# JJanai/back2future

Measured on AMD Instinct MI355X. Metric: frame-triplets/sec at 3x1024x1920, higher is better.
Workload: dtype f32; 1 GPU; BASELINE.json configs[4] per-GPU share: batch=16 synthetic 3x1024x1920 triplets per GPU, random-init pwc.lua weights (Ours-Hard shape), outputs flow + occ + est[3]; batch_per_gpu=16, global_batch=16, height=1024, width=1920, parallelism=dp1: independent triplets per rank, one RCCL weight broadcast at init, hip_graph=True

## Files before the change

### back2future_amd/_lib.py

```python
import ctypes as C
import os

import numpy as np

_HERE = os.path.dirname(os.path.abspath(__file__))
SO_PATH = os.environ.get("B2F_LIB") or os.path.join(_HERE, "libb2f.so")
_lib = None

c_float_p = C.POINTER(C.c_float)


class LossGradOpts(C.Structure):
    _fields_ = [("smooth_flow", C.c_double), ("const_vel", C.c_double), ("pme", C.c_double), ("smooth_occ", C.c_double),
                ("prior_occ", C.c_double), ("level_weights", C.c_double * 7), ("size_average", C.c_int)]


c_grad_opts_p = C.POINTER(LossGradOpts)


class LossGradFtOpts(C.Structure):
    _fields_ = LossGradOpts._fields_ + [("smooth_second_order", C.c_int), ("pme_criterion", C.c_int), ("pme_alpha", C.c_double),
                                        ("pme_beta", C.c_double), ("pme_gamma", C.c_double)]


# ... 336 lines not shown
    "b2f_op_cv_variant": (C.c_int, [C.c_void_p, C.c_int, C.c_int, C.c_int, C.c_int, C.c_int]),
    "b2f_op_conv_first": (C.c_int, [C.c_void_p, c_float_p, C.c_int, C.c_int, C.c_int, C.c_int, c_float_p, c_float_p, c_float_p]),
    "b2f_op_conv_head16": (C.c_int, [C.c_void_p, c_float_p, C.c_int, C.c_int, C.c_int, c_float_p, c_float_p, c_float_p, c_float_p, c_float_p]),
    "b2f_op_upsample_flow2x": (C.c_int, [C.c_void_p, c_float_p, C.c_int, C.c_int, C.c_int, c_float_p]),
    "b2f_op_image_scale": (C.c_int, [C.c_void_p, c_float_p, C.c_int, C.c_int, C.c_int, C.c_int, c_float_p, C.c_int, C.c_int]),
    "b2f_op_upsample_flow2x_ex": (C.c_int, [C.c_void_p, c_float_p, C.c_int, C.c_int, C.c_int, C.c_int, C.c_int, c_float_p]),
    "b2f_op_softmax_nearest4": (C.c_int, [C.c_void_p, c_float_p, C.c_int, C.c_int, C.c_int, C.c_int, c_float_p]),
    "b2f_op_avgpool2": (C.c_int, [C.c_void_p, c_float_p, C.c_int, C.c_int, C.c_int, C.c_int, c_float_p]),
    "b2f_op_pack_input": (C.c_int, [C.c_void_p, c_float_p, C.c_int, C.c_int, C.c_int, C.c_int, c_float_p]),
    "b2f_op_warp_image": (C.c_int, [C.c_void_p, C.c_int, C.c_void_p, C.c_int, C.c_int, c_float_p, C.c_float, C.c_int, C.c_int, C.c_int, c_float_p]),
    "b2f_op_conv_first_seq": (C.c_int, [C.c_void_p, C.c_void_p, C.c_int, C.c_int, C.c_int, C.c_int, c_float_p, c_float_p, c_float_p]),
    "b2f_op_layout": (C.c_int, [C.c_void_p, C.c_int, c_float_p, C.c_int, C.c_int, C.c_int, C.c_int, C.c_int, c_float_p]),
    "b2f_op_graph_put_channels": (C.c_int, [C.c_void_p, c_float_p, C.c_int, C.c_int, C.c_int, C.c_int, C.c_int, c_float_p, C.c_int, C.c_int]),
    "b2f_op_graph_costvol": (C.c_int, [C.c_void_p, c_float_p, c_float_p, c_float_p, C.c_int, C.c_int, C.c_int, C.c_int, C.c_int, C.c_int,
                                       c_float_p, C.c_int, c_float_p, C.c_int]),
    "b2f_op_graph_warp": (C.c_int, [C.c_void_p, c_float_p, C.c_int, c_float_p, C.c_float, C.c_int, C.c_int, C.c_int, c_float_p]),
    "b2f_op_graph_add_flow": (C.c_int, [C.c_void_p, c_float_p, c_float_p, C.c_longlong]),
    "b2f_op_graph_scale": (C.c_int, [C.c_void_p, c_float_p, C.c_longlong, C.c_float]),
    "b2f_op_graph_softmax_nearest": (C.c_int, [C.c_void_p, c_float_p, C.c_int, C.c_int, C.c_int, C.c_int, c_float_p]),
    "b2f_op_expf": (C.c_int, [C.c_void_p, c_float_p, C.c_longlong, c_float_p]),
    "b2f_arena_check": (C.c_int, [C.c_void_p, C.POINTER(C.c_int), C.POINTER(C.c_longlong)]),
    "b2f_guard_selftest": (C.c_int, [C.c_void_p, C.c_int]),
    "b2f_arena_plan": (C.c_int, [C.c_int, C.c_int, C.c_int, C.c_int, C.c_int, C.POINTER(C.c_longlong), C.c_int, C.POINTER(C.c_longlong)]),
}


class B2FError(RuntimeError):
    pass


def lib():
    global _lib
    if _lib is None:
        if not os.path.exists(SO_PATH):
            raise B2FError("%s is missing: build it with `python -m back2future_amd.build` "
                           "(there is no CPU fallback for the computeFlow path)" % SO_PATH)
        L = C.CDLL(SO_PATH)
        for name, (res, args) in SIGNATURES.items():
            fn = getattr(L, name)
            fn.restype = res
            fn.argtypes = args
        _lib = L
    return _lib


def check(rc):
# ... 11 lines not shown
```

### back2future_amd/back2future.py

```python
import ctypes as C
import weakref

import numpy as np

from . import _lib

meanstd = {"mean": [0.485, 0.456, 0.406], "std": [0.229, 0.224, 0.225]}
occ_threshold = 0.6666

IN_NORMALIZED, IN_UNIT, IN_U8 = 0, 1, 2
RGB_PLANAR, RGB_PACKED = 0, 1
STREAM_WARP, STREAM_PAST = 1, 2
SCORE_PIXELS, SCORE_EPE_Q20, SCORE_OUTLIERS, SCORE_OCC, SCORE_NONFINITE, SCORE_WORDS = 0, 4, 8, 12, 21, 22
PHOTO_INSIDE, PHOTO_OUTSIDE, PHOTO_CHARB_Q30, PHOTO_SQ_Q30, PHOTO_OCHARB_Q30, PHOTO_WEIGHT_Q30, PHOTO_NONFINITE, PHOTO_WORDS = 0, 2, 4, 6, 8, 10, 12, 14
LOSS_PIXELS, LOSS_SMOOTH_FLOW_Q30, LOSS_SMOOTH_PAST_Q30, LOSS_CONST_VEL_Q30, LOSS_SMOOTH_OCC_Q30, LOSS_PRIOR_OCC_Q30 = 0, 1, 2, 3, 4, 5
LOSS_PHOTO_INSIDE, LOSS_PHOTO_OUTSIDE, LOSS_PHOTO_OCHARB_Q30, LOSS_PHOTO_NONFINITE, LOSS_NONFINITE, LOSS_WORDS = 6, 8, 10, 12, 14, 16
LOSS_LEVEL_WEIGHTS = (0.005, 0.01, 0.02, 0.08, 0.32, 0.64, 1.28)
LOSS_WEIGHTS = {"smooth_flow": 1.0, "const_vel": 1.0, "pme": 1.0, "smooth_occ": 0.1, "prior_occ": 0.1}
LOSS_FT_SMOOTH2_FLOW_Q30, LOSS_FT_SMOOTH2_PAST_Q30, LOSS_FT_PHOTO_OGX_Q30, LOSS_FT_PHOTO_OGY_Q30 = 16, 17, 18, 20
LOSS_FT_SMOOTH2_NONFINITE, LOSS_FT_GRAD_NONFINITE, LOSS_FT_WORDS = 22, 23, 24
LOSS_SSIM_Q30, LOSS_SSIM_L1N_Q30, LOSS_SSIM_NONFINITE, LOSS_SSIM_RANGE_USED, LOSS_SSIM_RANGE_OWN, LOSS_SSIM_WORDS = 16, 18, 20, 22, 24, 32
SSIM_RANGE_BATCH, SSIM_RANGE_IMAGE, SSIM_RANGE_GIVEN = 0, 1, 2
SSIM_ALPHA = {"OSSIM": 1.0, "OSSIML1": 0.85}
LOSS_PLAIN_L1_Q30, LOSS_PLAIN_SQ_Q30, LOSS_PLAIN_SSIM_Q30, LOSS_PLAIN_L1N_Q30, LOSS_PLAIN_SSIM_NONFINITE = 16, 18, 20, 22, 24
# ... 1443 lines not shown

        entry = _grad_entry("b2f_multi_forward_loss_grad", options)
        fn = lambda h, xp, n, H, W, fsc, op, lp, gp, ng, outs, *tail: entry(h, xp, n, H, W, fsc, op, lp, gp, ng, *tail)
        L = no.value // (5 if pf.value else 4)
        grad, loss, _ = _forward_loss_grad(fn, self._h, x, flow_scale, options, shapes, L, want_loss, False,
                                           _grad_range_args(options, ssim_range, L, "MultiModel.forwardLossGrad", batch_ok=False))
        return (grad, loss) if want_loss else grad


ARENA_BUFFERS = (["img", "tmp"] + ["cs[%d]" % l for l in range(2, 8)] + ["U[%d]" % l for l in range(3, 7)] + ["UB[%d]" % l for l in range(3, 7)]
                 + ["cv"] + ["d[%d]" % i for i in range(1, 6)] + ["fs", "bfs", "logits", "u2", "flow_planar"] + ["ds[%d]" % k for k in range(2, 6)])


def arena_plan(B, H, W, full=False, past_flow=False, seq=False, stream=False, want_past=False, arena_guard=0):
    off, total = (C.c_longlong * 40)(), C.c_longlong()
    flags = (1 if full else 0) | (2 if past_flow else 0) | (4 if seq else 0) | (8 if stream else 0) | (16 if want_past else 0)
    n = _lib.lib().b2f_arena_plan(int(arena_guard), int(B), int(H), int(W), flags, off, 40, C.byref(total))
    if n < 0:
        _lib.check(1)
    assert n == len(ARENA_BUFFERS)
    return dict(zip(ARENA_BUFFERS, list(off)[:n])), total.value


def shard_range(n, rank, world):
    lo, hi = C.c_int(), C.c_int()
    _lib.check(_lib.lib().b2f_shard_range(int(n), int(rank), int(world), C.byref(lo), C.byref(hi)))
    return lo.value, hi.value


def init(opt=None, device=0):
    opt = opt or "Ours-Soft-ft-KITTI"
    model = Model(opt, device)

    def computeFlow(im1, im2, im3):
        return model.computeFlow(im1, im2, im3)

    computeFlow.model = model
    return computeFlow
```

### back2future_amd/csrc/b2f_api.hip

```cpp
#include "b2f_ctx.h"

#include <cctype>
#include <cmath>
#include <cstdio>
#include <cstdlib>

using namespace b2f;

static thread_local std::string g_err;
namespace b2f {
int api_fail(const std::string &m)
{
    g_err = m;
    return 1;
}
const std::string &api_error() { return g_err; }

ConvSeg cp8_seg(const float *ptr, int C, size_t hw)
{
    ConvSeg sgm;
    sgm.ptr = ptr;
    sgm.img_stride = (long)(hw * (size_t)((C + 7) / 8 * 8));
    sgm.chunk_stride = (long)(hw * 8);
    sgm.pix_stride = 8;
// ... 415 lines not shown
        if (o.wino1d && p.has(K_W1B) && blocks > 0 && w1b_supported(L)) {
            ch.kernel = K_W1B;
            ch.w1b_blocks = blocks;
        } else if (o.wino6 && p.has(K_WINO6) && H * W >= o.wino6_min_pixels && wino6_supported(L)) {
            ch.kernel = K_WINO6;
        }
    }
    return ch;
}

}

int b2f::launch_layer(b2f_ctx *c, hipStream_t s, bool prof, const PackedConv &p, const float *wpk, const KernelOpts &o, int cur_batch, ConvLaunch &L)
{
    for (int i = 0; i < p.nseg; ++i) L.seg[i].nchunks = p.chunks[i];
    if (p.nseg == 1) L.seg[1] = L.seg[0], L.seg[1].nchunks = 0;
    L.nseg = p.nseg;
    L.cout = p.cout;
    L.Ho = (L.H + 2 - 3) / L.stride + 1;
    L.Wo = (L.W + 2 - 3) / L.stride + 1;
    L.tiles_per_block = o.s2_tiles_per_block;
    L.w4_persist = o.wino4_persistent;
    L.w8 = o.wino8;
    L.bf16_direct = o.bf16_direct;
    auto weights = [&](ConvKernel k) { return p.has(k) ? wpk + p.pk[k].w_off : nullptr; };
    auto bias = [&](ConvKernel k) { return p.has(k) ? wpk + p.pk[k].b_off : nullptr; };
    L.wpk_bf6 = weights(K_BF6); L.bias_bf6 = bias(K_BF6);
    L.wpk_s2b = weights(K_S2B); L.bias_s2b = bias(K_S2B);
    L.wpk_w1b = weights(K_W1B); L.bias_w1b = bias(K_W1B);
    L.wpk_w6 = weights(K_WINO6); L.bias_w6 = bias(K_WINO6);
    const KernelChoice ch = choose_kernel(p, o, cur_batch, L);
    const PackedConv::Packing &q = p.pk[ch.f2x2 ? K_WINO2 : p.base];
    L.wpk = wpk + q.w_off;
    L.bias = wpk + q.b_off;
    L.nt = q.nt;
    L.nblk = q.nblk;
    L.nsplit = ch.nsplit;
    L.w1b_nblk = ch.w1b_blocks;
#if B2F_EXPERIMENTS
    if (!ch.f2x2) { L.wpk_split = weights(K_WINO4S); L.wpk_split2 = weights(K_WINO2S); }
    L.w4_hybrid = o.wino4_hybrid;
#endif
    const KernelRow &k = kKernels[ch.kernel];
    char name[48];
    if (c->profile_layers)
        snprintf(name, sizeof name, "conv%s_%dto%d_%dx%d", (B2F_EXPERIMENTS && ch.kernel == K_C16 && o.bf16_direct) ? "B16" : k.tag[L.stride - 1],
// ... 304 lines not shown
    OPT_SYNC = 2,
    OPT_EXP_ONLY = 4,
    OPT_ARENA = 8,
};
struct OptRow {
    const char *name;
    int b2f_ctx::*member;
    int flags;
    int repack;
};
const OptRow kOptions[] = {
    {"use_graph", &b2f_ctx::use_graph, OPT_ENV, 0},
    {"host_graph", &b2f_ctx::host_graph, OPT_ENV, 0},
    {"profile", &b2f_ctx::profile, OPT_ENV, 0},
    {"profile_layers", &b2f_ctx::profile_layers, OPT_ENV, 0},
    {"corr_variant", &b2f_ctx::corr_variant, OPT_ENV | OPT_SYNC, 0},
    {"corr_ablate", &b2f_ctx::corr_ablate, OPT_ENV | OPT_SYNC, 0},
    {"bf16_direct", &b2f_ctx::bf16_direct, OPT_ENV | OPT_SYNC, 0},
    {"bf16_conv", &b2f_ctx::bf16_conv, OPT_ENV | OPT_SYNC, 1},
    {"bf16_conv_min_pixels", &b2f_ctx::bf16_conv_min_pixels, OPT_SYNC, 0},
    {"wino1d", &b2f_ctx::wino1d, OPT_ENV | OPT_SYNC, 2},
    {"wino6", &b2f_ctx::wino6, OPT_ENV | OPT_SYNC, 3},
    {"wino6_min_pixels", &b2f_ctx::wino6_min_pixels, OPT_ENV | OPT_SYNC, 0},
    {"wino2_split", &b2f_ctx::wino2_split, OPT_ENV | OPT_SYNC | OPT_EXP_ONLY, 4},
    {"wino4_split", &b2f_ctx::wino4_split, OPT_ENV | OPT_SYNC | OPT_EXP_ONLY, 5},
    {"wino4_hybrid", &b2f_ctx::wino4_hybrid, OPT_ENV | OPT_SYNC | OPT_EXP_ONLY, 5},
    {"s2_tiles_per_block", &b2f_ctx::s2_tiles_per_block, OPT_ENV | OPT_SYNC, 0},
    {"wino4_persistent", &b2f_ctx::wino4_persistent, OPT_ENV | OPT_SYNC, 0},
    {"s2_loader", &b2f_ctx::s2_loader, OPT_ENV | OPT_SYNC, 0},
    {"s2_tile_groups", &b2f_ctx::s2_tile_groups, OPT_ENV | OPT_SYNC, 0},
    {"wino_split_pixels", &b2f_ctx::wino_split_pixels, OPT_ENV | OPT_SYNC, 0},
    {"wino8", &b2f_ctx::wino8, OPT_ENV | OPT_SYNC, 0},
    {"wino4_min_pixels", &b2f_ctx::wino4_min_pixels, OPT_ENV | OPT_SYNC, 0},
    {"adaptive_kernels", &b2f_ctx::adaptive_kernels, OPT_ENV | OPT_SYNC, 0},
    {"op_wino_split", &b2f_ctx::op_wino_split, OPT_ENV, 0},
    {"op_gradw_partials", &b2f_ctx::op_gradw_partials, OPT_ENV, 0},
    {"op_hole_fill", &b2f_ctx::op_hole_fill, 0, 0},
    {"host_subbatch_pixels", nullptr, OPT_ENV, 0},
    {"host_threads", &b2f_ctx::host_threads, OPT_ENV, 0},
    {"host_u8", &b2f_ctx::host_u8, OPT_ENV, 0},
    {"host_ramp", &b2f_ctx::host_ramp, OPT_ENV, 0},
    {"debug_fail_next", &b2f_ctx::debug_fail_next, 0, 0},
    {"arena_guard", &b2f_ctx::arena_guard, OPT_ARENA, 0},
    {"arena_fill", &b2f_ctx::arena_fill, OPT_ARENA, 0},
};

// ... 6 lines not shown

bool reads_packing(const b2f_ctx *c, int group)
{
    for (const OptRow &r : kOptions)
        if (r.repack == group && (r.member == &b2f_ctx::bf16_conv ? c->*r.member >= 2 : c->*r.member != 0)) return true;
    return false;
}

const char *experiment_value(const OptRow &r, int value)
{
    if (B2F_EXPERIMENTS) return nullptr;
    if (r.member == &b2f_ctx::corr_variant && (value == 2 || value == 4 || value == 6 || value == 8))
        return "b2f_set_option: corr_variant 2 / 4 / 6 / 8 are experiment kernels: build with `python -m back2future_amd.build --experiments`";
    if (r.member == &b2f_ctx::bf16_direct && value == 1)
        return "b2f_set_option: bf16_direct = 1 (the 16 -> 16 layer alone on the bf16 pipe) is an experiment: build with `python -m back2future_amd.build --experiments`";
    return nullptr;
}

}

extern "C" {

const char *b2f_last_error(void) { return g_err.c_str(); }
int b2f_version(void) { return 1015; }

long long b2f_param_count(int past_flow) { return param_count(past_flow != 0); }

int b2f_random_weights(unsigned long long seed, int past_flow, float gain, float *out, long long n) try
{
    if (!out || n != param_count(past_flow != 0)) return fail("b2f_random_weights: bad buffer size");
    random_weights(seed, past_flow != 0, gain, out);
    return 0;
}
B2F_CATCH("b2f_random_weights")

int b2f_load_t7(const char *path, float *out, long long cap, long long *n, int *past_flow) try
{
    std::vector<float> flat;
    bool past = false;
    std::string err;
    if (!path) return fail("b2f_load_t7: null path");
    if (!load_t7(path, flat, past, err)) return fail("b2f_load_t7: " + err);
    if (n) *n = (long long)flat.size();
    if (past_flow) *past_flow = past ? 1 : 0;
    if (out) {
        if (cap < (long long)flat.size()) return fail("b2f_load_t7: output buffer too small");
        memcpy(out, flat.data(), flat.size() * sizeof(float));
// ... 230 lines not shown
        if (r->member == &b2f_ctx::arena_guard && (value < 0 || value % 64)) return fail("b2f_set_option: arena_guard is a count of floats, a multiple of 64");
        if (r->member == &b2f_ctx::arena_fill && value != 0 && value != 1) return fail("b2f_set_option: arena_fill is 0 or 1");
        HIPCHK(hipSetDevice(c->device));
        HIPCHK(hipDeviceSynchronize());
        drop_graphs(c);
        if (c->arena) HIPCHK(hipFree(c->arena));
        c->arena = nullptr;
        c->arena_floats = 0;
        c->guards.clear();
        c->arena_layout[0] = 0;
    }
    const bool had = r->repack && reads_packing(c, r->repack);
    c->*r->member = value;
    if (r->repack && had != reads_packing(c, r->repack)) CHK(b2f_commit_weights(c));
    return 0;
}
B2F_CATCH("b2f_set_option")

int b2f_get_option(const b2f_ctx *c, const char *key, int *value) try
{
    if (!c || !key || !value) return fail("b2f_get_option: null argument");
    const OptRow *r = find_option(key);
    if (!strcmp(key, "experiments")) *value = B2F_EXPERIMENTS;
    else if (!r) return fail(std::string("b2f_get_option: unknown key ") + key);
    else if (!r->member) *value = (int)std::min<long long>(c->host_subbatch_pixels, 0x7fffffff);
    else *value = c->*r->member;
    return 0;
}
B2F_CATCH("b2f_get_option")

int b2f_synchronize(b2f_ctx *c) try
{
    if (!c) return fail("b2f_synchronize: null context");
    HIPCHK(hipSetDevice(c->device));
    HIPCHK(hipStreamSynchronize(c->stream));
    return 0;
}
B2F_CATCH("b2f_synchronize")

int b2f_profile_reset(b2f_ctx *c) try
{
    if (!c) return fail("b2f_profile_reset: null context");
    CHK(prof_collect(c));
    std::fill(c->prof_ms.begin(), c->prof_ms.end(), 0.0);
    std::fill(c->prof_n.begin(), c->prof_n.end(), 0);
    return 0;
// ... 677 lines not shown
B2F_CATCH("b2f_guard_selftest")

int b2f_arena_plan(int arena_guard, int B, int H, int W, int flags, long long *offsets, int cap, long long *total) try
{
    if (!offsets || cap < 33 || arena_guard < 0 || arena_guard % 64) { fail("b2f_arena_plan: bad argument"); return -1; }
    if (check_shape(B, H, W)) return -1;
    const Plan p = make_plan((size_t)arena_guard, B, H, W, (flags & 1) != 0, (flags & 2) != 0, (flags & 4) != 0, (flags & 8) != 0, (flags & 16) != 0);
    int n = 0;
    offsets[n++] = (long long)p.img;
    offsets[n++] = (long long)p.tmp;
    for (int l = 2; l <= 7; ++l) offsets[n++] = (long long)p.cs[l];
    for (int l = 3; l <= 6; ++l) offsets[n++] = (long long)p.U[l];
    for (int l = 3; l <= 6; ++l) offsets[n++] = (long long)p.UB[l];
    offsets[n++] = (long long)p.cv;
    for (int i = 1; i <= 5; ++i) offsets[n++] = (long long)p.d[i];
    for (size_t o : {p.fs, p.bfs, p.logits, p.u2, p.flow_planar}) offsets[n++] = (long long)o;
    for (int k = 2; k <= 5; ++k) offsets[n++] = (long long)p.ds[k];
    if (total) *total = (long long)p.total;
    return n;
}
catch (const std::exception &e) { fail(std::string("b2f_arena_plan: ") + e.what()); return -1; }
catch (...) { fail("b2f_arena_plan: unknown exception"); return -1; }

}

int b2f::pointer_kind(const void *p)
{
    hipPointerAttribute_t a;
    if (hipPointerGetAttributes(&a, p) != hipSuccess) {
        (void)hipGetLastError();
        return 0;
    }
    if (a.type == hipMemoryTypeDevice || a.type == hipMemoryTypeManaged || a.type == hipMemoryTypeArray) return -1;
    return a.type == hipMemoryTypeHost ? 1 : 0;
}

int b2f::check_device_pointers(const std::string &w, const b2f_ctx *c, const char *use, const void *const *ptrs, size_t count, size_t aligned)
{
    uintptr_t bits = 0;
    for (size_t i = 0; i < aligned; ++i) bits |= (uintptr_t)ptrs[i];
    if (bits & 15) return fail(w + ": device buffers must be 16-byte aligned");
    if (!c) return fail(w + ": null context");
    HIPCHK(hipSetDevice(c->device));
    for (size_t i = 0; i < count; ++i)
        if (ptrs[i] && host_memory(ptrs[i])) return fail(w + ": host memory passed to a device entry point (use " + use + ")");
    return 0;
// ... 18 lines not shown
```

### back2future_amd/csrc/b2f_ctx.h

```cpp
#pragma once
#include "../../include/b2f.h"

#include <algorithm>
#include <atomic>
#include <condition_variable>
#include <cstring>
#include <deque>
#include <exception>
#include <map>
#include <memory>
#include <mutex>
#include <string>
#include <thread>
#include <tuple>
#include <vector>

#include "b2f_host.h"
#include "b2f_internal.h"

namespace b2f {

int api_fail(const std::string &m);
const std::string &api_error();

// ... 22 lines not shown
    int cout = 0;
    ConvKernel base = K_DIRECT;
    struct Packing {
        size_t w_off = 0, b_off = 0;
        int nt = 0, nblk = 0;
    } pk[K_COUNT];
    bool has(ConvKernel k) const { return pk[k].nblk != 0; }
    int nchunks() const { return chunks[0] + (nseg > 1 ? chunks[1] : 0); }
};

struct KernelOpts {
    int wino8 = 1;
    int wino_split_pixels = 512;
    int wino4_min_pixels = 4096;
    int adaptive_kernels = -1;
    int bf16_direct = 2;
    int bf16_conv_min_pixels = 65536;
    int bf16_conv = 1;
    int wino2_split = 0;
    int wino4_hybrid = 0;
    int wino4_split = 0;
    int wino6 = 1;
    int wino6_min_pixels = 16384;
    int wino1d = 0;
    int s2_tile_groups = 1;
    int s2_loader = 1;
    int wino4_persistent = 1;
    int s2_tiles_per_block = 0;
};

struct ProfEvent {
    int name;
    hipEvent_t a, b;
};

struct GraphKey {
    const void *in;
    float *flow, *occ, *est3;
    int kind, B, H, W;
    int rule;
    int seq;
    const void *ring = nullptr;
    int phase = 0;
    float *past = nullptr;
    bool operator<(const GraphKey &o) const
    {
// ... 566 lines not shown
```

### back2future_amd/csrc/b2f_internal.h

```cpp
#pragma once
#include <hip/hip_runtime.h>
#ifndef B2F_EXPERIMENTS
#define B2F_EXPERIMENTS 0
#endif
#include <atomic>
#include <cstdint>

namespace b2f {

constexpr int kLevels = 7, kLst = 3, kWin = 9, kND = 2 * kWin * kWin;
constexpr int kFeat[8] = {0, 3, 16, 32, 64, 96, 128, 192};
constexpr int kDec[7] = {0, 128, 128, 96, 64, 32, 2};
constexpr int kCvRec = 168;
constexpr int kCvChunks = 21;
constexpr int kImgC = 8;
constexpr int kCK = 8;

struct ConvSeg {
    const float *ptr;
    long img_stride;
    long chunk_stride;
    int pix_stride;
    int nchunks;
};
// ... 12 lines not shown
    int nimg;
    int leaky;
    long long *trace;
    int nb0;
    int nsplit;
    int w8 = 1;
    int w4_persist = 1;
    int tiles_per_block = 0;
    int w4_hybrid = 0;
    const void *wpk_split2 = nullptr;
    const void *wpk_bf6 = nullptr;
    const float *bias_bf6 = nullptr;
    int bf16_direct = 0;
    const void *wpk_split = nullptr;
    const void *wpk_w1b = nullptr;
    const float *bias_w1b = nullptr;
    const void *wpk_s2b = nullptr;
    const float *bias_s2b = nullptr;
    int w1b_nblk = 0;
    const void *wpk_w6 = nullptr;
    const float *bias_w6 = nullptr;
    unsigned w6_mul[3] = {0, 0, 0};
    int w6_sh[3] = {0, 0, 0};
};
hipError_t launch_conv3x3(const ConvLaunch &p, hipStream_t s);
size_t conv_wpk_floats(int cin_chunks, int nt, int nblk);
void conv_choose_tiles(int cout, int *nt, int *nblk);
void conv_pack_weights(const float *w, const float *b, int Co, int Ci, const int *cin_map,
                       int cin_chunks, int nt, int nblk, float *wpk, float *bpk);

hipError_t launch_conv3x3_c16(const ConvLaunch &p, hipStream_t s);
hipError_t launch_conv3x3_c16b(const ConvLaunch &p, hipStream_t s);
size_t c16_wpk_floats();
void c16_pack_weights(const float *w, const float *b, int Ci, const int *cin_map, float *wpk, float *bpk);
bool convb_supported(const ConvLaunch &p);
hipError_t launch_conv3x3_bf6(const ConvLaunch &p, hipStream_t s);
int convb_nblk(int cout);
size_t convb_wpk_floats(int cin_chunks, int cout);
void convb_pack_weights(const float *w, const float *b, int Co, int Ci, const int *cin_map, int cin_chunks, float *wpk, float *bpk);
bool s2b_supported(const ConvLaunch &p);
hipError_t launch_conv3x3_s2b(const ConvLaunch &p, hipStream_t s);
int s2b_ntiles(int cout);
size_t s2b_wpk_floats(int cin_chunks, int cout);
void s2b_pack_weights(const float *w, const float *b, int Co, int Ci, const int *cin_map, int cin_chunks, float *wpk, float *bpk);
bool w1b_supported(const ConvLaunch &p);
hipError_t launch_conv3x3_w1b(const ConvLaunch &p, hipStream_t s);
int w1b_nblk(int cout);
size_t w1b_wpk_floats(int cin_chunks, int cout);
void w1b_pack_weights(const float *w, const float *b, int Co, int Ci, const int *cin_map, int cin_chunks, float *wpk, float *bpk);
bool wino6_supported(const ConvLaunch &p);
hipError_t launch_conv3x3_wino6(const ConvLaunch &p, hipStream_t s);
int wino6_nblk(int cout);
size_t wino6_wpk_floats(int cin_chunks, int cout);
void wino6_pack_weights(const float *w, const float *b, int Co, int Ci, const int *cin_map, int cin_chunks, float *wpk, float *bpk);
struct HeadLaunch {
    const float *in;
    long in_img_stride, in_chunk_stride;
    int in_pix_stride;
    int H1, W1;
    const float *w1, *b1, *w2, *b2;
    float *out;
    long out_img_stride, out_chunk_stride;
    int out_pix_stride;
    int Ho, Wo, nimg;
    int rows_per_block, nsy, nsx;
    long long *trace = nullptr;
};
bool head16_supported(const HeadLaunch &p);
hipError_t launch_conv_head16(HeadLaunch p, hipStream_t s);
bool c16s2_supported(const ConvLaunch &p);
hipError_t launch_conv3x3_c16s2(const ConvLaunch &p, hipStream_t s);
size_t c16s2_wpk_floats();
void c16s2_pack_weights(const float *w, const float *b, int Ci, const int *cin_map, float *wpk, float *bpk);
hipError_t launch_conv_narrow2(const ConvLaunch &p, hipStream_t s);
// ... 199 lines not shown
```

### back2future_amd/csrc/b2f_wino6.hip

```cpp
#include "b2f_internal.h"

#include <cstdio>
#include <cstdlib>
#include <vector>

namespace b2f {

namespace wino6 {
typedef float f32x4 __attribute__((ext_vector_type(4)));
typedef float f32x2 __attribute__((ext_vector_type(2)));
typedef unsigned long long u64;

constexpr int OH = 12, OW = 48;
constexpr int PH = OH + 2, PW = OW + 2;
constexpr int RP = 56;
constexpr int PL = 808;
constexpr int SLOT_BYTES = 4 * PL * 8;
constexpr int SLOT_STRIDE = 32768;
constexpr int SLOT_F2 = SLOT_STRIDE / 8;
constexpr int BIAS_OFF = SLOT_BYTES;
constexpr int BIAS_MAX = (SLOT_STRIDE - SLOT_BYTES) / 4;
constexpr int X_OFF = SLOT_STRIDE + SLOT_BYTES;
constexpr int XPS = 2176;
constexpr int X_BYTES = 48 * XPS;
// ... 175 lines not shown
                const unsigned vo = (ok && oy + 2 * i < p.Ho) ? ooff + (unsigned)(i * rowstep) : 0xfffffff0u;
                __builtin_amdgcn_raw_buffer_store_b128(__builtin_bit_cast(__attribute__((ext_vector_type(4))) unsigned, v), o_rsrc, (int)vo, 0, W6_OUT_AUX);
            }
#pragma unroll
            for (int b = 3 * rr; b < 3 * rr + 3 && b < 8; ++b) {
                W6_ACC_RESET(b, 2 * ps);
                W6_ACC_RESET(b, 2 * ps + 1);
            }
            __builtin_amdgcn_sched_barrier(0);
        }
        if (W6_ABLATE & 32) {
#pragma unroll
            for (int b = 0; b < 8; ++b) {
                W6_ACC_RESET(b, 2 * ps);
                W6_ACC_RESET(b, 2 * ps + 1);
            }
        }
        W6_T(4 + 3 * ps);
    }
#undef W6_ACC_RESET
}

template <int NT>
__global__ __launch_bounds__(512) void conv3x3_wino6(const ConvLaunch p)
{
    using namespace wino6;
    static_assert(NT == 4 || NT == 2, "64 or 32 outputs per block");
    constexpr int NSTEP = 4 * NT;
    constexpr int SPS = 16 / NSTEP;
    constexpr int LAG = SPS;
    constexpr int UCN = UC * NT / 4;
    extern __shared__ __attribute__((aligned(16))) char smem[];
    f32x2 *raw2 = reinterpret_cast<f32x2 *>(smem);

    const int tid = threadIdx.x;
    const int lane = tid & 63;
    const int wave = __builtin_amdgcn_readfirstlane(tid >> 6);

    const int tiles_x = (p.Wo + OW - 1) / OW, tiles_y = (p.Ho + OH - 1) / OH;
    const int total = tiles_x * tiles_y * p.nimg * p.nblk;
    const int G = gridDim.x;
    const int nchunks = p.seg[0].nchunks + (p.nseg > 1 ? p.seg[1].nchunks : 0);
    if ((int)blockIdx.x >= total) return;

    for (int i = tid; i < p.nblk * 64; i += 512) reinterpret_cast<float *>(smem + BIAS_OFF)[i] = p.bias[p.nb0 * 64 + i];

    int rA = 0, rB = 0;
    float rc1, rc2, rc3, rc4, rc5;
    switch (wave) {
    case 0: rB = -1; rc1 = 5.25f; rc2 = -5.25f; rc3 = -1.f; rc4 = 0.f; rc5 = 0.f; break;
    case 1: rc1 = 1.f; rc2 = -4.25f; rc3 = 1.f; rc4 = -4.25f; rc5 = 1.f; break;
    case 2: rc1 = 1.f; rc2 = -4.25f; rc3 = -1.f; rc4 = 4.25f; rc5 = -1.f; break;
    case 3: rc1 = .25f; rc2 = -1.25f; rc3 = .5f; rc4 = -2.5f; rc5 = 2.f; break;
    case 4: rc1 = .25f; rc2 = -1.25f; rc3 = -.5f; rc4 = 2.5f; rc5 = -2.f; break;
    case 5: rc1 = 4.f; rc2 = -5.f; rc3 = 2.f; rc4 = -2.5f; rc5 = .5f; break;
    case 6: rc1 = 4.f; rc2 = -5.f; rc3 = -2.f; rc4 = 2.5f; rc5 = -.5f; break;
    default: rA = 1; rc1 = 0.f; rc2 = 0.f; rc3 = -1.f; rc4 = 5.25f; rc5 = -5.25f; break;
    }
    const f32x2 pc12 = {rc1, rc2}, pc34 = {rc3, rc4}, pc5x = {rc5, rc5};
    const int t_t = lane & 15, t_kq = lane >> 4;
    const int t_b = t_kq * PL + (6 * (t_t >> 3)) * RP + (t_t & 7);
    const int t_iA = t_b + rA * RP, t_iB = t_b + rB * RP;

    const int s_idx = min(tid, NSTG - 1) >> 1, s_h = tid & 1;
    const int s_r5 = s_idx / PW, s_px = s_idx - s_r5 * PW;
    const int s_slot = (2 * s_h) * PL + s_r5 * RP + colpos(s_px);
// ... 178 lines not shown
            if (!(W6_ABLATE & 8)) W6_MFMA(PP_, st, 0);                                              \
            __builtin_amdgcn_sched_barrier(0);                                                      \
            W6_SLOT_LDS(SPS * st, PP_);                                                             \
            __builtin_amdgcn_sched_barrier(0);                                                      \
            if (!(W6_ABLATE & 8)) W6_MFMA(PP_, st, 1);                                              \
            __builtin_amdgcn_sched_barrier(0);                                                      \
            if (SPS == 2) W6_SLOT_VALU(2 * st + 1, PP_);                                            \
            if (!(W6_ABLATE & 4)) W6_B_LOAD(st + W6_RING - 1);                                      \
            W6_SLOT_VMEM(SPS * st);                                                                 \
            if (SPS == 2) W6_SLOT_VMEM(2 * st + 1);                                                 \
            __builtin_amdgcn_sched_barrier(0);                                                      \
            if (!(W6_ABLATE & 8)) W6_MFMA(PP_, st, 2);                                              \
            if (SPS == 2) {                                                                         \
                __builtin_amdgcn_sched_barrier(0);                                                  \
                W6_SLOT_LDS(2 * st + 1, PP_);                                                       \
                __builtin_amdgcn_sched_barrier(0);                                                  \
            }                                                                                       \
            if (!(W6_ABLATE & 8)) W6_MFMA(PP_, st, 3);                                              \
            __builtin_amdgcn_sched_barrier(0);                                                      \
        }                                                                                           \
        if (!(W6_ABLATE & 16)) W6_LDS_BARRIER();                                                    \
    } while (0)

    int v_cur = blockIdx.x;
    W6_DECODE(v_cur, cur_nb, cur_img, cur_ox0, cur_oy0);
    if (W6_NB_DELAY > 0 && p.nblk > 1 && ((cur_nb - p.nb0) & 1)) __builtin_amdgcn_s_sleep(W6_NB_DELAY);
    W6_MASKS(cur_ox0, cur_oy0, mk);
    W6_BASES(cur_img, cur_ox0, cur_oy0, ld_b0, ld_b1);
    nxt_b0 = ld_b0; nxt_b1 = ld_b1;
    has_next = false;
    nxt_nb = cur_nb; nxt_img = cur_img; nxt_ox0 = cur_ox0; nxt_oy0 = cur_oy0;
    mk_n[0] = mk[0]; mk_n[1] = mk[1]; mk_n[2] = mk[2];
    bo_c = cur_nb * nchunks * UC;
    bo_n = bo_c + UCN;
    {
        W6_LOAD_STREAM();
        f32x4 keep[3];
#pragma unroll
        for (int i = 0; i < 3; ++i) keep[i] = sr[i];
        W6_LOAD_STREAM();
#pragma unroll
        for (int u = 0; u < W6_RING - 1; ++u) W6_B_LOAD(u);
        W6_RAW_WRITE(raw2 + SLOT_F2);
#pragma unroll
        for (int i = 0; i < 3; ++i) sr[i] = keep[i];
        W6_RAW_WRITE(raw2);
        W6_LOAD_STREAM();
    }
    __syncthreads();
#pragma unroll
    for (int col = 0; col < 8; ++col) { W6_ROW_READ(col, raw2); W6_ROW_FMA(col); }
#pragma unroll
    for (int part = 0; part < 4; ++part) W6_COLPASS(part, 0);
    W6_LDS_BARRIER();

    const bool tr_on = W6_TRACE && p.trace && p.nb0 >= 0 && blockIdx.x == 40 && (wave == 0 || wave == 4) && p.w8 == 77;
    long long *tr_buf = W6_TRACE ? (p.trace ? p.trace : reinterpret_cast<long long *>(p.out)) + (tr_on ? (wave >> 2) * 128 : 256) : nullptr;
    int tr_item = 0;
    int c = 0;
    bool more = true;
#define W6_ITEM_START()                                                                             \
    do {                                                                                            \
        has_next = v_cur + G < total;                                                               \
        if (has_next) {                                                                             \
            W6_DECODE(v_cur + G, nxt_nb, nxt_img, nxt_ox0, nxt_oy0);                                \
            W6_MASKS(nxt_ox0, nxt_oy0, mk_n);                                                       \
            W6_BASES(nxt_img, nxt_ox0, nxt_oy0, nxt_b0, nxt_b1);                                    \
        }                                                                                           \
    } while (0)
#define W6_ACC_INIT()                                                                               \
    do {                                                                                            \
        _Pragma("unroll") for (int b = 0; b < 8; ++b)                                               \
            _Pragma("unroll") for (int mt = 0; mt < NT; ++mt) acc[b][mt] = f32x4{0.f, 0.f, 0.f, 0.f}; \
         \
         \
        {                                                                                           \
            int z__ = 0;                                                                            \
            asm volatile("" : "+v"(z__));                                                           \
            const int q4__ = (int)__builtin_amdgcn_mbcnt_hi(~0u, __builtin_amdgcn_mbcnt_lo(~0u, (unsigned)z__)) >> 4; \
// ... 32 lines not shown
        if (!more) break;
        W6_RUN(1);
    }
#undef W6_RUN
#undef W6_ACC_INIT
#undef W6_ITEM_START
#undef W6_PERIOD
#undef W6_SLOT_VMEM
#undef W6_SLOT_LDS
#undef W6_SLOT_VALU
#undef W6_MFMA
#undef W6_B_LOAD
#undef W6_COLPASS
#undef W6_ROW_FMA
#undef W6_ROW_READ
#undef W6_RAW_WRITE
#undef W6_LOAD_STREAM
#undef W6_BASES
#undef W6_MASKS
#undef W6_DECODE
#undef W6_DIV
}

bool wino6_supported(const ConvLaunch &p)
{
    if (p.stride != 1 || p.H != p.Ho || p.W != p.Wo) return false;
    if (p.nseg > 1 && p.seg[1].pix_stride != p.seg[0].pix_stride) return false;
    if (((p.out_pix_stride | (int)p.out_chunk_stride) & 3) != 0 || (p.cout & 3) != 0) return false;
    const int nchunks = p.seg[0].nchunks + (p.nseg > 1 ? p.seg[1].nchunks : 0);
    if (nchunks < 4) return false;
    if ((long)wino6_nblk(p.cout) * 64 > wino6::BIAS_MAX) return false;
    if ((double)wino6_nblk(p.cout) * nchunks * wino6::UC >= 2147483648.0) return false;
    for (int i = 0; i < p.nseg; ++i)
        if ((double)p.seg[i].nchunks * (double)p.seg[i].chunk_stride * 4.0 + 9.0 * p.W * p.seg[0].pix_stride * 4.0 >= 2147483648.0) return false;
    if ((double)((p.cout + 7) / 8) * (double)p.out_chunk_stride * 4.0 + (double)p.Ho * p.Wo * p.out_pix_stride * 4.0 >= 2147483648.0) return false;
    return (double)p.H * p.W * p.seg[0].pix_stride * 4.0 < 2147483648.0;
}

template <int NT>
static hipError_t launch_wino6_t(const ConvLaunch &p, int nb0, int nblk, hipStream_t s)
{
    using namespace wino6;
    static LdsOnce once;
    const int slot = current_device_slot();
    if (hipError_t e = once.ensure(reinterpret_cast<const void *>(&conv3x3_wino6<NT>), LDS_BYTES, slot)) return e;
    ConvLaunch q = p;
    q.wpk = reinterpret_cast<const float *>(p.wpk_w6);
    q.bias = p.bias_w6;
    q.nb0 = nb0;
    q.nblk = nblk;
    w6_div_magic(nblk, &q.w6_mul[0], &q.w6_sh[0]);
    w6_div_magic((p.Wo + OW - 1) / OW, &q.w6_mul[1], &q.w6_sh[1]);
    w6_div_magic((p.Ho + OH - 1) / OH, &q.w6_mul[2], &q.w6_sh[2]);
    q.trace = nullptr;
#if W6_TRACE
    static long long *trace_dev = nullptr;
    static int traced = 0;
    const int tr_want = getenv("B2F_WINO_TRACE") ? atoi(getenv("B2F_WINO_TRACE")) : 0;
    const int nch = p.seg[0].nchunks + (p.nseg > 1 ? p.seg[1].nchunks : 0);
    const int tr_nt = getenv("B2F_WINO_TRACE_NT") ? atoi(getenv("B2F_WINO_TRACE_NT")) : 4;
    const bool do_trace = NT == tr_nt && tr_want == nch && traced < 1 && p.H * p.W >= 256 * 480;
    if (do_trace) {
        if (!trace_dev) hipMalloc(&trace_dev, 512 * sizeof(long long));
        hipMemsetAsync(trace_dev, 0, 512 * sizeof(long long), s);
    }
    if (!trace_dev) hipMalloc(&trace_dev, 512 * sizeof(long long));
    q.trace = trace_dev;
    q.w8 = do_trace ? 77 : 0;
#endif
    const long items = (long)((p.Wo + OW - 1) / OW) * ((p.Ho + OH - 1) / OH) * p.nimg * nblk;
    const int pcap = p.w4_persist > 1 ? p.w4_persist : persistent_block_cap(slot);
    const int grid = (int)(items < pcap ? items : pcap);
    hipLaunchKernelGGL((conv3x3_wino6<NT>), dim3((unsigned)grid), dim3(512), LDS_BYTES, s, q);
#if W6_TRACE
    if (do_trace) {
        ++traced;
        long long h[256];
        hipStreamSynchronize(s);
        hipMemcpy(h, trace_dev, sizeof h, hipMemcpyDeviceToHost);
        for (int w = 0; w < 2; ++w) {
            fprintf(stderr, "wino6<%d> trace, block 40 wave %d, %d chunks: per item, cycles: K loop (per chunk) | dump 0 | barrier | rounds 0 | barrier + dump 1 | barrier | rounds 1 | item switch\n", NT, 4 * w, nch);
            for (int it = 0; it < 6; ++it) {
                const long long *t = h + w * 128 + it * 16;
                if (!t[0]) continue;
                fprintf(stderr, "  item %d: %7lld (%5lld) | %5lld | %5lld | %5lld | %5lld | %5lld | %5lld | %5lld\n", it, t[1] - t[0], (t[1] - t[0]) / nch, t[2] - t[1], t[3] - t[2], t[4] - t[3],
                        NT == 4 ? t[5] - t[4] : 0, NT == 4 ? t[6] - t[5] : 0, NT == 4 ? t[7] - t[6] : 0, t[8] - t[NT == 4 ? 7 : 4]);
            }
        }
    }
#endif
    return hipGetLastError();
}

hipError_t launch_conv3x3_wino6(const ConvLaunch &p, hipStream_t s)
{
    if (!wino6_supported(p) || !p.wpk_w6) return hipErrorInvalidValue;
    const int rem = p.cout % 64, n64 = p.cout / 64 + (rem > 32 ? 1 : 0);
    hipError_t e = hipSuccess;
    if (n64 > 0) e = launch_wino6_t<4>(p, 0, n64, s);
    if (e == hipSuccess && rem > 0 && rem <= 32) e = launch_wino6_t<2>(p, p.cout / 64, 1, s);
    return e;
}

int wino6_nblk(int cout) { return (cout + 63) / 64; }

size_t wino6_wpk_floats(int cin_chunks, int cout)
{
    const int rem = cout % 64;
    return (size_t)(cout / 64) * cin_chunks * (wino6::UC / 4) + (rem > 32 ? (size_t)cin_chunks * (wino6::UC / 4) : rem > 0 ? (size_t)cin_chunks * (wino6::UC / 8) : 0);
}

void wino6_pack_weights(const float *w, const float *b, int Co, int Ci, const int *cin_map, int cin_chunks, float *wpk, float *bpk)
{
    static const double G[8][3] = {{1, 0, 0},
                                   {-2.0 / 9, -2.0 / 9, -2.0 / 9},
                                   {-2.0 / 9, 2.0 / 9, -2.0 / 9},
                                   {1.0 / 90, 1.0 / 45, 2.0 / 45},
                                   {1.0 / 90, -1.0 / 45, 2.0 / 45},
                                   {32.0 / 45, 16.0 / 45, 8.0 / 45},
                                   {32.0 / 45, -16.0 / 45, 8.0 / 45},
// ... 42 lines not shown
```

### include/b2f.h

```cpp
#ifndef B2F_H
#define B2F_H

#include <stddef.h>
#include <stdint.h>

#ifdef __cplusplus
extern "C" {
#endif

#if defined(__GNUC__)
#define B2F_API __attribute__((visibility("default")))
#else
#define B2F_API
#endif

typedef struct b2f_ctx b2f_ctx;

B2F_API const char *b2f_last_error(void);

B2F_API int b2f_version(void);

B2F_API int b2f_init(const char *name_or_path, int device, b2f_ctx **out);
B2F_API int b2f_init_ex(const char *name_or_path, int device, const char *graph_opts, b2f_ctx **out);
B2F_API void b2f_destroy(b2f_ctx *ctx);
// ... 488 lines not shown

B2F_API int b2f_op_upsample_flow2x_ex(b2f_ctx *ctx, const float *x, int ps, int B, int h, int w, int planar, float *y);
B2F_API int b2f_op_softmax_nearest4(b2f_ctx *ctx, const float *logits, int ps, int B, int h, int w, float *out);
B2F_API int b2f_op_avgpool2(b2f_ctx *ctx, const float *x, int nimg, int H, int W, int C, float *y);
B2F_API int b2f_op_pack_input(b2f_ctx *ctx, const float *x, int normalize, int B, int H, int W, float *img);
B2F_API int b2f_op_warp_image(b2f_ctx *ctx, int which, const void *in, int in_kind, int frame, const float *flow, float k, int B,
                      int H, int W, float *out);
B2F_API int b2f_op_conv_first_seq(b2f_ctx *ctx, const void *x, int in_kind, int T, int H, int W, const float *w, const float *b, float *y);
B2F_API int b2f_op_layout(b2f_ctx *ctx, int which, const float *in, int C, int pix_stride, int B, int h, int w, float *out);
B2F_API int b2f_op_graph_put_channels(b2f_ctx *ctx, const float *src, int kind, int src_chunks, int C, int B, int hw, float *dst,
                              int dst_chunks, int c_off);
B2F_API int b2f_op_graph_costvol(b2f_ctx *ctx, const float *ref, const float *frmF, const float *frmB, int chunks, int C, int B, int h,
                         int w, int win, float *dstJ, int chunksJ, float *dstS, int chunksS);
B2F_API int b2f_op_graph_warp(b2f_ctx *ctx, const float *img, int chunks, const float *flow, float k, int B, int h, int w, float *out);
B2F_API int b2f_op_graph_add_flow(b2f_ctx *ctx, float *fs, const float *u, long long npix);
B2F_API int b2f_op_graph_scale(b2f_ctx *ctx, float *p, long long n, float k);
B2F_API int b2f_op_graph_softmax_nearest(b2f_ctx *ctx, const float *logits, int B, int h, int w, int f, float *out);
B2F_API int b2f_op_expf(b2f_ctx *ctx, const float *x, long long n, float *y);


B2F_API int b2f_arena_check(b2f_ctx *ctx, int *buffer_index, long long *offset);
B2F_API int b2f_guard_selftest(b2f_ctx *ctx, int which);
B2F_API int b2f_arena_plan(int arena_guard, int B, int H, int W, int flags, long long *offsets, int cap, long long *total);

#ifdef __cplusplus
}
#endif
#endif
```

Measured before the change: 848.6 triplets/s.

## Fuse wino6 64-wide and 32-wide output-channel passes into one persistent launch

When a Winograd F6 conv layer's output channels split into 64-wide blocks plus a remainder of 32 or fewer, both parts now run in a single kernel launch. The persistent block budget is divided between the two variants in proportion to estimated per-item costs. This is meant to remove the serial tail where the small 32-wide launch runs alone on an underused GPU after the 64-wide launch drains. It relies on the hardcoded cost constants being accurate, and a bad split could leave one side as the straggler.

```diff
diff --git a/back2future_amd/_lib.py b/back2future_amd/_lib.py
--- a/back2future_amd/_lib.py
+++ b/back2future_amd/_lib.py
@@ -382,6 +382,7 @@
     "b2f_arena_check": (C.c_int, [C.c_void_p, C.POINTER(C.c_int), C.POINTER(C.c_longlong)]),
     "b2f_guard_selftest": (C.c_int, [C.c_void_p, C.c_int]),
     "b2f_arena_plan": (C.c_int, [C.c_int, C.c_int, C.c_int, C.c_int, C.c_int, C.POINTER(C.c_longlong), C.c_int, C.POINTER(C.c_longlong)]),
+    "b2f_wino6_blocks": (C.c_int, [C.c_longlong, C.c_longlong, C.c_int, C.POINTER(C.c_int), C.POINTER(C.c_int)]),
 }
 
 
diff --git a/back2future_amd/back2future.py b/back2future_amd/back2future.py
--- a/back2future_amd/back2future.py
+++ b/back2future_amd/back2future.py
@@ -1489,6 +1489,14 @@
     return dict(zip(ARENA_BUFFERS, list(off)[:n])), total.value
 
 
+def wino6_blocks(items64, items32, cap):
+    g64, g32 = C.c_int(), C.c_int()
+    r = _lib.lib().b2f_wino6_blocks(int(items64), int(items32), int(cap), C.byref(g64), C.byref(g32))
+    if r < 0:
+        _lib.check(1)
+    return (g64.value, g32.value) if r else None
+
+
 def shard_range(n, rank, world):
     lo, hi = C.c_int(), C.c_int()
     _lib.check(_lib.lib().b2f_shard_range(int(n), int(rank), int(world), C.byref(lo), C.byref(hi)))
diff --git a/back2future_amd/csrc/b2f_api.hip b/back2future_amd/csrc/b2f_api.hip
--- a/back2future_amd/csrc/b2f_api.hip
+++ b/back2future_amd/csrc/b2f_api.hip
@@ -461,6 +461,7 @@
     L.tiles_per_block = o.s2_tiles_per_block;
     L.w4_persist = o.wino4_persistent;
     L.w8 = o.wino8;
+    L.w6_one_launch = o.wino6_one_launch;
     L.bf16_direct = o.bf16_direct;
     auto weights = [&](ConvKernel k) { return p.has(k) ? wpk + p.pk[k].w_off : nullptr; };
     auto bias = [&](ConvKernel k) { return p.has(k) ? wpk + p.pk[k].b_off : nullptr; };
@@ -811,6 +812,7 @@
     {"wino1d", &b2f_ctx::wino1d, OPT_ENV | OPT_SYNC, 2},
     {"wino6", &b2f_ctx::wino6, OPT_ENV | OPT_SYNC, 3},
     {"wino6_min_pixels", &b2f_ctx::wino6_min_pixels, OPT_ENV | OPT_SYNC, 0},
+    {"wino6_one_launch", &b2f_ctx::wino6_one_launch, OPT_ENV | OPT_SYNC, 0},
     {"wino2_split", &b2f_ctx::wino2_split, OPT_ENV | OPT_SYNC | OPT_EXP_ONLY, 4},
     {"wino4_split", &b2f_ctx::wino4_split, OPT_ENV | OPT_SYNC | OPT_EXP_ONLY, 5},
     {"wino4_hybrid", &b2f_ctx::wino4_hybrid, OPT_ENV | OPT_SYNC | OPT_EXP_ONLY, 5},
@@ -863,7 +865,7 @@
 extern "C" {
 
 const char *b2f_last_error(void) { return g_err.c_str(); }
-int b2f_version(void) { return 1015; }
+int b2f_version(void) { return 1016; }
 
 long long b2f_param_count(int past_flow) { return param_count(past_flow != 0); }
 
@@ -1140,6 +1142,11 @@
     if (!c || !key || !value) return fail("b2f_get_option: null argument");
     const OptRow *r = find_option(key);
     if (!strcmp(key, "experiments")) *value = B2F_EXPERIMENTS;
+    else if (!strcmp(key, "captured_graphs")) {
+        int n = 0;
+        for (const auto &kv : c->graphs) n += kv.second ? 1 : 0;
+        *value = n;
+    }
     else if (!r) return fail(std::string("b2f_get_option: unknown key ") + key);
     else if (!r->member) *value = (int)std::min<long long>(c->host_subbatch_pixels, 0x7fffffff);
     else *value = c->*r->member;
@@ -1863,6 +1870,12 @@
 catch (const std::exception &e) { fail(std::string("b2f_arena_plan: ") + e.what()); return -1; }
 catch (...) { fail("b2f_arena_plan: unknown exception"); return -1; }
 
+int b2f_wino6_blocks(long long items64, long long items32, int cap, int *g64, int *g32)
+{
+    if (!g64 || !g32 || items64 < 1 || items32 < 1 || cap < 1 || items64 > (1ll << 40) || items32 > (1ll << 40)) { fail("b2f_wino6_blocks: bad argument"); return -1; }
+    return wino6_split_blocks((long)items64, (long)items32, cap, g64, g32) ? 1 : 0;
+}
+
 }
 
 int b2f::pointer_kind(const void *p)
diff --git a/back2future_amd/csrc/b2f_ctx.h b/back2future_amd/csrc/b2f_ctx.h
--- a/back2future_amd/csrc/b2f_ctx.h
+++ b/back2future_amd/csrc/b2f_ctx.h
@@ -68,6 +68,7 @@
     int wino4_split = 0;
     int wino6 = 1;
     int wino6_min_pixels = 16384;
+    int wino6_one_launch = 1;
     int wino1d = 0;
     int s2_tile_groups = 1;
     int s2_loader = 1;
diff --git a/back2future_amd/csrc/b2f_internal.h b/back2future_amd/csrc/b2f_internal.h
--- a/back2future_amd/csrc/b2f_internal.h
+++ b/back2future_amd/csrc/b2f_internal.h
@@ -58,6 +58,7 @@
     const float *bias_w6 = nullptr;
     unsigned w6_mul[3] = {0, 0, 0};
     int w6_sh[3] = {0, 0, 0};
+    int w6_one_launch = 1;
 };
 hipError_t launch_conv3x3(const ConvLaunch &p, hipStream_t s);
 size_t conv_wpk_floats(int cin_chunks, int nt, int nblk);
@@ -86,6 +87,7 @@
 void w1b_pack_weights(const float *w, const float *b, int Co, int Ci, const int *cin_map, int cin_chunks, float *wpk, float *bpk);
 bool wino6_supported(const ConvLaunch &p);
 hipError_t launch_conv3x3_wino6(const ConvLaunch &p, hipStream_t s);
+bool wino6_split_blocks(long items64, long items32, int cap, int *g64, int *g32);
 int wino6_nblk(int cout);
 size_t wino6_wpk_floats(int cin_chunks, int cout);
 void wino6_pack_weights(const float *w, const float *b, int Co, int Ci, const int *cin_map, int cin_chunks, float *wpk, float *bpk);
diff --git a/back2future_amd/csrc/b2f_wino6.hip b/back2future_amd/csrc/b2f_wino6.hip
--- a/back2future_amd/csrc/b2f_wino6.hip
+++ b/back2future_amd/csrc/b2f_wino6.hip
@@ -221,7 +221,7 @@
 }
 
 template <int NT>
-__global__ __launch_bounds__(512) void conv3x3_wino6(const ConvLaunch p)
+__device__ __forceinline__ void wino6_block(const ConvLaunch &p, const int bid, const int G)
 {
     using namespace wino6;
     static_assert(NT == 4 || NT == 2, "64 or 32 outputs per block");
@@ -238,9 +238,8 @@
 
     const int tiles_x = (p.Wo + OW - 1) / OW, tiles_y = (p.Ho + OH - 1) / OH;
     const int total = tiles_x * tiles_y * p.nimg * p.nblk;
-    const int G = gridDim.x;
     const int nchunks = p.seg[0].nchunks + (p.nseg > 1 ? p.seg[1].nchunks : 0);
-    if ((int)blockIdx.x >= total) return;
+    if (bid >= total) return;
 
     for (int i = tid; i < p.nblk * 64; i += 512) reinterpret_cast<float *>(smem + BIAS_OFF)[i] = p.bias[p.nb0 * 64 + i];
 
@@ -465,7 +464,7 @@
         if (!(W6_ABLATE & 16)) W6_LDS_BARRIER();                                                    \
     } while (0)
 
-    int v_cur = blockIdx.x;
+    int v_cur = bid;
     W6_DECODE(v_cur, cur_nb, cur_img, cur_ox0, cur_oy0);
     if (W6_NB_DELAY > 0 && p.nblk > 1 && ((cur_nb - p.nb0) & 1)) __builtin_amdgcn_s_sleep(W6_NB_DELAY);
     W6_MASKS(cur_ox0, cur_oy0, mk);
@@ -497,7 +496,7 @@
     for (int part = 0; part < 4; ++part) W6_COLPASS(part, 0);
     W6_LDS_BARRIER();
 
-    const bool tr_on = W6_TRACE && p.trace && p.nb0 >= 0 && blockIdx.x == 40 && (wave == 0 || wave == 4) && p.w8 == 77;
+    const bool tr_on = W6_TRACE && p.trace && p.nb0 >= 0 && bid == 40 && (wave == 0 || wave == 4) && p.w8 == 77;
     long long *tr_buf = W6_TRACE ? (p.trace ? p.trace : reinterpret_cast<long long *>(p.out)) + (tr_on ? (wave >> 2) * 128 : 256) : nullptr;
     int tr_item = 0;
     int c = 0;
@@ -576,6 +575,19 @@
 #undef W6_DIV
 }
 
+template <int NT>
+__global__ __launch_bounds__(512) void conv3x3_wino6(const ConvLaunch p)
+{
+    wino6_block<NT>(p, (int)blockIdx.x, (int)gridDim.x);
+}
+
+__global__ __launch_bounds__(512) void conv3x3_wino6_both(const ConvLaunch p, const ConvLaunch p32, const int g64)
+{
+    const int b = (int)blockIdx.x;
+    if (b < g64) wino6_block<4>(p, b, g64);
+    else wino6_block<2>(p32, b - g64, (int)gridDim.x - g64);
+}
+
 bool wino6_supported(const ConvLaunch &p)
 {
     if (p.stride != 1 || p.H != p.Ho || p.W != p.Wo) return false;
@@ -591,13 +603,9 @@
     return (double)p.H * p.W * p.seg[0].pix_stride * 4.0 < 2147483648.0;
 }
 
-template <int NT>
-static hipError_t launch_wino6_t(const ConvLaunch &p, int nb0, int nblk, hipStream_t s)
+static ConvLaunch wino6_args(const ConvLaunch &p, int nb0, int nblk)
 {
     using namespace wino6;
-    static LdsOnce once;
-    const int slot = current_device_slot();
-    if (hipError_t e = once.ensure(reinterpret_cast<const void *>(&conv3x3_wino6<NT>), LDS_BYTES, slot)) return e;
     ConvLaunch q = p;
     q.wpk = reinterpret_cast<const float *>(p.wpk_w6);
     q.bias = p.bias_w6;
@@ -607,6 +615,17 @@
     w6_div_magic((p.Wo + OW - 1) / OW, &q.w6_mul[1], &q.w6_sh[1]);
     w6_div_magic((p.Ho + OH - 1) / OH, &q.w6_mul[2], &q.w6_sh[2]);
     q.trace = nullptr;
+    return q;
+}
+
+template <int NT>
+static hipError_t launch_wino6_t(const ConvLaunch &p, int nb0, int nblk, hipStream_t s)
+{
+    using namespace wino6;
+    static LdsOnce once;
+    const int slot = current_device_slot();
+    if (hipError_t e = once.ensure(reinterpret_cast<const void *>(&conv3x3_wino6<NT>), LDS_BYTES, slot)) return e;
+    ConvLaunch q = wino6_args(p, nb0, nblk);
 #if W6_TRACE
     static long long *trace_dev = nullptr;
     static int traced = 0;
@@ -646,10 +665,60 @@
     return hipGetLastError();
 }
 
+#ifndef W6_COST64
+#define W6_COST64 435
+#endif
+#ifndef W6_COST32
+#define W6_COST32 340
+#endif
+constexpr long long kW6Cost64 = W6_COST64, kW6Cost32 = W6_COST32;
+
+bool wino6_split_blocks(long items64, long items32, int cap, int *g64, int *g32)
+{
+    *g64 = *g32 = 0;
+    if (items64 < 1 || items32 < 1 || cap < 2) return false;
+    if (items64 + items32 <= cap) {
+        *g64 = (int)items64;
+        *g32 = (int)items32;
+        return true;
+    }
+    const long long w64 = items64 * kW6Cost64, w32 = items32 * kW6Cost32;
+    const int unit = (cap % 8 == 0 && cap >= 16) ? 8 : 1;
+    long long a = (cap / unit * w64 + (w64 + w32) / 2) / (w64 + w32) * unit;
+    a = a < unit ? unit : a > cap - unit ? cap - unit : a;
+    if (a > items64) a = items64;
+    long long b = cap - a;
+    if (b > items32) {
+        b = items32;
+        a = cap - b < items64 ? cap - b : items64;
+    }
+    *g64 = (int)a;
+    *g32 = (int)b;
+    return true;
+}
+
+static hipError_t launch_wino6_both(const ConvLaunch &p, int n64, int g64, int g32, int slot, hipStream_t s)
+{
+    using namespace wino6;
+    static LdsOnce once;
+    if (hipError_t e = once.ensure(reinterpret_cast<const void *>(&conv3x3_wino6_both), LDS_BYTES, slot)) return e;
+    const ConvLaunch q = wino6_args(p, 0, n64), q32 = wino6_args(p, p.cout / 64, 1);
+    hipLaunchKernelGGL(conv3x3_wino6_both, dim3((unsigned)(g64 + g32)), dim3(512), LDS_BYTES, s, q, q32, g64);
+    return hipGetLastError();
+}
+
 hipError_t launch_conv3x3_wino6(const ConvLaunch &p, hipStream_t s)
 {
+    using namespace wino6;
     if (!wino6_supported(p) || !p.wpk_w6) return hipErrorInvalidValue;
     const int rem = p.cout % 64, n64 = p.cout / 64 + (rem > 32 ? 1 : 0);
+    if (!W6_TRACE && p.w6_one_launch && n64 > 0 && rem > 0 && rem <= 32) {
+        const int slot = current_device_slot();
+        const long tiles = (long)((p.Wo + OW - 1) / OW) * ((p.Ho + OH - 1) / OH) * p.nimg;
+        const int pcap = p.w4_persist > 1 ? p.w4_persist : persistent_block_cap(slot);
+        int g64 = 0, g32 = 0;
+        if (wino6_split_blocks(tiles * n64, tiles, pcap, &g64, &g32)) return launch_wino6_both(p, n64, g64, g32, slot, s);
+    }
     hipError_t e = hipSuccess;
     if (n64 > 0) e = launch_wino6_t<4>(p, 0, n64, s);
     if (e == hipSuccess && rem > 0 && rem <= 32) e = launch_wino6_t<2>(p, p.cout / 64, 1, s);
diff --git a/include/b2f.h b/include/b2f.h
--- a/include/b2f.h
+++ b/include/b2f.h
@@ -534,6 +534,7 @@
 B2F_API int b2f_arena_check(b2f_ctx *ctx, int *buffer_index, long long *offset);
 B2F_API int b2f_guard_selftest(b2f_ctx *ctx, int which);
 B2F_API int b2f_arena_plan(int arena_guard, int B, int H, int W, int flags, long long *offsets, int cap, long long *total);
+B2F_API int b2f_wino6_blocks(long long items64, long long items32, int cap, int *g64, int *g32);
 
 #ifdef __cplusplus
 }
```

Measured after the change: 853.4 triplets/s, median of 6. No clear change (+0.6%).
